# nonl4331/raytracing-rust

Measured on NVIDIA B200. Metric: Mrays/s, higher is better.
Workload: dtype f32

## Files before the change

### raytracing-rust_b200/csrc/context.cu

```cuda
#include <cstdarg>
#include <cstring>
#include <new>

#include "ptb_internal.h"

namespace ptb {

static thread_local std::string g_create_error;

int32_t set_error(Ctx* c, int32_t code, const char* fmt, ...) {
  char buf[512];
  va_list ap;
  va_start(ap, fmt);
  vsnprintf(buf, sizeof buf, fmt, ap);
  va_end(ap);
  if (c) c->last_error = buf;
  else g_create_error = buf;
  return code;
}
int32_t check_cuda(Ctx* c, cudaError_t e, const char* what) {
  if (e == cudaSuccess) return PTB_OK;
  const int32_t code = e == cudaErrorMemoryAllocation ? PTB_ERR_OOM : PTB_ERR_CUDA;
  return set_error(c, code, "CUDA error %d (%s) in %s", (int)e, cudaGetErrorString(e), what);
}
// ... 32 lines not shown
  if (!out) return PTB_ERR_INVALID;
  *out = nullptr;
  int n = 0;
  cudaError_t e = cudaGetDeviceCount(&n);
  if (e != cudaSuccess || n == 0)
    return set_error(nullptr, PTB_ERR_CUDA, "no CUDA device available (%s); ptb200 has no CPU fallback",
                     e == cudaSuccess ? "device count is 0" : cudaGetErrorString(e));
  if (device < 0 || device >= n) return set_error(nullptr, PTB_ERR_INVALID, "device %d out of range [0,%d)", device, n);
  ptb_ctx* ctx = new (std::nothrow) ptb_ctx();
  if (!ctx) return PTB_ERR_OOM;
  Ctx* c = &ctx->c;
  c->device = device;
  auto fail = [&](cudaError_t err, const char* what) {
    int32_t rc = set_error(nullptr, PTB_ERR_CUDA, "%s: %s", what, cudaGetErrorString(err));
    delete ctx;
    return rc;
  };
  if ((e = cudaSetDevice(device)) != cudaSuccess) return fail(e, "cudaSetDevice");
  cudaDeviceProp prop;
  if ((e = cudaGetDeviceProperties(&prop, device)) != cudaSuccess) return fail(e, "cudaGetDeviceProperties");
  if (prop.major < 10) {
    int32_t rc = set_error(nullptr, PTB_ERR_CUDA, "device %d is sm_%d%d; ptb200 is built for sm_100a only", device, prop.major,
                           prop.minor);
    delete ctx;
    return rc;
  }
  c->sm_count = prop.multiProcessorCount;
  c->dev.trace_burst = 8;
  c->dev.trace_fetch_threshold = 8;
  c->dev.trace_prim_bias = 0;
  if (const char* e = getenv("PTB_TRACE_PRIM_BIAS")) { int v = atoi(e); if (v >= 0 && v <= 32) c->dev.trace_prim_bias = v; }
  if (const char* e = getenv("PTB_TRACE_BURST")) { int v = atoi(e); if (v >= 1 && v <= 64) c->dev.trace_burst = v; }
  if (const char* e = getenv("PTB_TRACE_FETCH")) { int v = atoi(e); if (v >= 1 && v <= 32) c->dev.trace_fetch_threshold = v; }
  if ((e = cudaStreamCreateWithFlags(&c->stream, cudaStreamNonBlocking)) != cudaSuccess) return fail(e, "cudaStreamCreate");
  c->own_stream = true;
  if ((e = cudaEventCreate(&c->ev_a)) != cudaSuccess) return fail(e, "cudaEventCreate");
  if ((e = cudaEventCreate(&c->ev_b)) != cudaSuccess) return fail(e, "cudaEventCreate");
  if ((e = cudaEventCreate(&c->ev_iter)) != cudaSuccess) return fail(e, "cudaEventCreate");
  *out = ctx;
  return PTB_OK;
}

int32_t ptb_destroy(ptb_ctx* ctx) {
  if (!ctx) return PTB_OK;
  Ctx* c = &ctx->c;
  cudaSetDevice(c->device);
  if (c->stream) cudaStreamSynchronize(c->stream);
  if (c->h_counters) cudaFreeHost(c->h_counters);
  if (c->h_sah) cudaFreeHost(c->h_sah);
  for (float* h : c->h_pass)
    if (h) cudaFreeHost(h);
  if (c->ev_a) cudaEventDestroy(c->ev_a);
  if (c->ev_b) cudaEventDestroy(c->ev_b);
  if (c->ev_iter) cudaEventDestroy(c->ev_iter);
  for (int b = 0; b < 2; ++b) {
    if (c->ev_in[b]) cudaEventDestroy(c->ev_in[b]);
    if (c->ev_kernel[b]) cudaEventDestroy(c->ev_kernel[b]);
    if (c->ev_out[b]) cudaEventDestroy(c->ev_out[b]);
  }
  for (cudaEvent_t e : c->ev_head_done) if (e) cudaEventDestroy(e);
  for (cudaEvent_t e : c->ev_tail_done) if (e) cudaEventDestroy(e);
  for (cudaEvent_t e : c->ev_ring) if (e) cudaEventDestroy(e);
  if (c->s_tail) { cudaStreamSynchronize(c->s_tail); cudaStreamDestroy(c->s_tail); }
  if (c->s_work2) { cudaStreamSynchronize(c->s_work2); cudaStreamDestroy(c->s_work2); }
  if (c->ev_fork) cudaEventDestroy(c->ev_fork);
  if (c->ev_join) cudaEventDestroy(c->ev_join);
// ... 514 lines not shown
```

### raytracing-rust_b200/csrc/lbvh_build.cu

```cuda
#include <cstdarg>
#include <cstring>

#include "ptb_internal.h"

namespace ptb {

__device__ __forceinline__ uint32_t float_flip(float f) {
  uint32_t u = __float_as_uint(f);
  return (u & 0x80000000u) ? ~u : (u | 0x80000000u);
}
__device__ __forceinline__ float float_unflip(uint32_t u) {
  return __uint_as_float((u & 0x80000000u) ? (u & 0x7FFFFFFFu) : ~u);
}
__device__ __forceinline__ uint32_t expand_bits10(uint32_t v) {
  v = (v * 0x00010001u) & 0xFF0000FFu;
  v = (v * 0x00000101u) & 0x0F00F00Fu;
  v = (v * 0x00000011u) & 0xC30C30C3u;
  v = (v * 0x00000005u) & 0x49249249u;
  return v;
}
__device__ __forceinline__ uint32_t quantise10(float c, float cmin, float ext) {
  float n = ext > 0.0f ? (c - cmin) / ext : 0.0f;
  float s = fminf(fmaxf(n * 1024.0f, 0.0f), 1023.0f);
  return (uint32_t)s;
// ... 752 lines not shown
  if (rc != PTB_OK) return rc;
  PTB_CUDA_TRY(c, cudaEventRecord(c->ev_b, st));
  PTB_CUDA_TRY(c, cudaStreamSynchronize(st));
  PTB_CUDA_TRY(c, cudaGetLastError());
  float ms = 0.f;
  cudaEventElapsedTime(&ms, c->ev_a, c->ev_b);
  c->stats.build_ms = ms;
  if (PTB_QNODES)
    for (int k = 0; k < 3; ++k) { c->dev.q_min[k] = h_qframe[k]; c->dev.q_step[k] = h_qframe[3 + k]; }
  c->dev.lights = c->d_lights.as<uint32_t>();
  c->dev.n_lights = nl;
  c->committed = true;
  return PTB_OK;
}

int32_t build_scene(Ctx* c, uint32_t build_flags) {
  if (build_flags & PTB_BUILD_REFIT) return refit_scene(c, build_flags);
  c->refittable = false;
  {
    int32_t rc = commit_tables(c);
    if (rc != PTB_OK) return rc;
  }
  const size_t ns = c->n_spheres, nt = c->n_tris;
  const size_t n = ns + nt;
  cudaStream_t st = c->stream;

  c->n_prims = n;
  c->n_nodes = n == 0 ? 0 : (n == 1 ? 1 : n - 1);
  c->dev.n_prims = (uint32_t)n;
  c->dev.n_lights = 0;
  c->dev.geom = nullptr; c->dev.normals = nullptr; c->dev.slot_prim = nullptr; c->dev.slot_mat = nullptr;
  c->dev.nodes = nullptr; c->dev.qnodes = nullptr; c->dev.lights = nullptr; c->dev.cw_nodes = nullptr;
  c->wide = false;
  if (n == 0) {
    c->committed = true;
    c->refittable = true;
    c->topo_spheres = ns;
    c->topo_tris = nt;
    c->stats.build_ms = 0.0;
    return PTB_OK;
  }

  DevBuf &raw_spheres = c->d_raw_spheres, &raw_tris = c->d_raw_tris;
  DevBuf &bmin = c->scratch[0], &bmax = c->scratch[1], &bounds = c->scratch[2], &keys_a = c->scratch[3], &keys_b = c->scratch[4],
         &vals_a = c->scratch[5], &vals_b = c->scratch[6], &hist = c->scratch[7], &leaf_parent = c->d_leaf_parent,
         &nbmin = c->scratch[9], &nbmax = c->scratch[10], &flags = c->scratch[11], &prim_slot = c->d_prim_slot,
         &d_light_prims = c->scratch[12], &d_light_tmp = c->scratch[13], &d_light_out = c->scratch[14], &d_qframe = c->scratch[15];
  const uint32_t n32 = (uint32_t)n, ns32 = (uint32_t)ns, nt32 = (uint32_t)nt;
  PTB_CUDA_TRY(c, bmin.reserve(n * 16));
  PTB_CUDA_TRY(c, bmax.reserve(n * 16));
  PTB_CUDA_TRY(c, bounds.reserve(12 * 4));
  PTB_CUDA_TRY(c, keys_a.reserve(n * 4));
  PTB_CUDA_TRY(c, keys_b.reserve(n * 4));
  PTB_CUDA_TRY(c, vals_a.reserve(n * 4));
  PTB_CUDA_TRY(c, vals_b.reserve(n * 4));
  PTB_CUDA_TRY(c, hist.reserve(radix_sort_hist_words(n32) * 4));
  PTB_CUDA_TRY(c, leaf_parent.reserve(n * 4));
  PTB_CUDA_TRY(c, nbmin.reserve(c->n_nodes * 16));
  PTB_CUDA_TRY(c, nbmax.reserve(c->n_nodes * 16));
  PTB_CUDA_TRY(c, flags.reserve(c->n_nodes * 4));
  PTB_CUDA_TRY(c, prim_slot.reserve(n * 4));
  PTB_CUDA_TRY(c, d_light_prims.reserve(n * 4));
  PTB_CUDA_TRY(c, d_light_tmp.reserve(n * 4));
  PTB_CUDA_TRY(c, d_light_out.reserve(8));
  PTB_CUDA_TRY(c, c->d_nodes.reserve(c->n_nodes * sizeof(BvhNode)));
  if (PTB_QNODES) PTB_CUDA_TRY(c, c->d_qnodes.reserve(c->n_nodes * 32));
// ... 81 lines not shown
    const int32_t rcw = build_wide(c, bi, final_prim.as<uint32_t>());
    if (rcw != PTB_OK) return rcw;
    slot_order = final_prim.as<uint32_t>();
    PTB_CUDA_TRY(c, cudaMemcpyAsync(c->d_prim_sorted.p, va, n * 4, cudaMemcpyDeviceToDevice, st));
  }
  k_gather<<<gn, T, 0, st>>>(raw_spheres.as<ptb_sphere>(), ns32, raw_tris.as<ptb_triangle>(), n32, slot_order,
                             c->d_materials.as<DevMaterial>(), (uint32_t)c->materials.size(), c->d_geom.as<float4>(),
                             c->d_normals.as<float4>(),
                             c->d_slot_mat.as<uint32_t>(), prim_slot.as<uint32_t>());
  c->stats.kernel_launches += 1;
  PTB_CUDA_TRY(c, cudaMemcpyAsync(c->d_morton.p, ka, n * 4, cudaMemcpyDeviceToDevice, st));
  PTB_CUDA_TRY(c, cudaMemcpyAsync(c->d_slot_prim.p, slot_order, n * 4, cudaMemcpyDeviceToDevice, st));
  uint32_t nl = 0;
  {
    const int32_t rcl = light_list(c, ns32, &nl);
    if (rcl != PTB_OK) return rcl;
  }
  PTB_CUDA_TRY(c, cudaEventRecord(c->ev_b, st));
  PTB_CUDA_TRY(c, cudaStreamSynchronize(st));
  PTB_CUDA_TRY(c, cudaGetLastError());
  float ms = 0.f;
  cudaEventElapsedTime(&ms, c->ev_a, c->ev_b);
  c->stats.build_ms = ms;

  c->dev.geom = c->d_geom.as<float4>();
  c->dev.normals = c->d_normals.as<float4>();
  c->dev.slot_prim = c->d_slot_prim.as<uint32_t>();
  c->dev.slot_mat = c->d_slot_mat.as<uint32_t>();
  c->dev.nodes = c->d_nodes.as<BvhNode>();
  c->dev.qnodes = (wide || !PTB_QNODES) ? nullptr : c->d_qnodes.as<uint4>();
  for (int k = 0; k < 3; ++k) { c->dev.q_min[k] = h_qframe[k]; c->dev.q_step[k] = h_qframe[3 + k]; }
  c->dev.cw_nodes = wide ? c->d_cw_nodes.as<CwNode>() : nullptr;
  c->wide = wide;
  c->sah = sah;
  if (!wide) c->n_cw_nodes = 0;
  c->dev.lights = c->d_lights.as<uint32_t>();
  c->dev.n_lights = nl;
  c->committed = true;
  c->refittable = true;
  c->topo_spheres = ns;
  c->topo_tris = nt;
  return PTB_OK;
}

}
```

### raytracing-rust_b200/csrc/ptb_common.cuh

```cuda
#pragma once
#include <cuda_runtime.h>
#include <stdint.h>

#include "../../include/ptb200.h"

namespace ptb {

#define PTB_DEV __device__ __forceinline__
#define PTB_HD __host__ __device__ __forceinline__

constexpr float kPi = 3.14159265358979323846f;
constexpr float kTau = 6.28318530717958647692f;
constexpr float kEpsRt = 3.0e-4f;
constexpr float kF32Eps = 1.1920929e-7f;
#ifndef PTB_QNODES
#define PTB_QNODES 0
#endif
constexpr uint32_t kSphereBit = 0x40000000u;
constexpr uint32_t kSlotMask = 0x3FFFFFFFu;
constexpr uint32_t kNone = 0xFFFFFFFFu;

struct v3 {
  float x, y, z;
};
// ... 231 lines not shown
    const float phi = atan2f(direction.y, direction.x) + kPi;
    const float theta = acosf(direction.z);
    const float uvx = phi / (2.0f * kPi), uvy = theta / kPi;
    const uint32_t dim0 = width - 1u, dim1 = height - 1u;
    const uint32_t x_pixel = sat_index((float)dim0 * uvx, dim0), y_pixel = sat_index((float)dim1 * uvy, dim1);
    const uint32_t index = 3u * (y_pixel * (dim0 + 1u) + x_pixel);
    return mk(words.f(index), words.f(index + 1u), words.f(index + 2u));
  }
  if (kind == PTB_TEX_PERLIN) return 0.5f * mk(1.0f, 1.0f, 1.0f) * (1.0f + perlin_noise(words, point));
  return mk(1.0f, 1.0f, 1.0f);
}

struct DevScene {
  const float4* geom;
  const float4* normals;
  const uint32_t* slot_prim;
  const uint32_t* slot_mat;
  const BvhNode* nodes;
  const uint4* qnodes;
  float q_min[3], q_step[3];
  const CwNode* cw_nodes;
  const DevMaterial* materials;
  const DevTexture* textures;
  const float* tex_data;
  const uint32_t* lights;
  uint32_t n_prims, n_lights;
  uint32_t sky_tex, sky_rx, sky_ry;
  const float* sky_ycdf;
  const float* sky_ypdf;
  const float* sky_xcdf;
  const float* sky_xpdf;
  v3 cam_origin, cam_lower_left, cam_horizontal, cam_vertical;
  int trace_burst, trace_fetch_threshold, trace_prim_bias;
};

}
```

### raytracing-rust_b200/csrc/ptb_coop.cuh

```cuda
#pragma once
#include "ptb_intersect.cuh"

namespace ptb {

constexpr uint32_t kCoopRays = 16;
constexpr uint32_t kCoopTagMask = 31u;
#ifndef PTB_COOP_CAP
#define PTB_COOP_CAP 1024
#endif
constexpr uint32_t kCoopCap = PTB_COOP_CAP;
constexpr uint32_t kCoopSoft = kCoopCap - 96u;

#ifdef PTB_TAIL_STATS
__device__ unsigned long long g_tail_stats[16] = {0, 0, 0, 0, 0, 0, 0, 0, 0, ~0ull, 0, 0, 0, 0, 0, 0};
#define PTB_TS(i, v) atomicAdd(&g_tail_stats[i], (unsigned long long)(v))
#else
#define PTB_TS(i, v) do { } while (0)
#endif

struct CoopRay {
  float ox, oy, oz, dx, dy, dz, shx, shy, shz;
  uint32_t swap_xz;
  float ax, ay, az, lx, ly, lz, hx, hy, hz;
  uint32_t exclude;
};
struct CoopWarp {
  unsigned long long best[kCoopRays];
  uint32_t ref[kCoopRays];
  CoopRay ray[kCoopRays];
  uint2 stack[kCoopCap];
};

PTB_DEV void coop_set_ray(const DevScene& sc, CoopWarp& cw, uint32_t j, const Ray& ray, float tmax, uint32_t exclude) {
  const BinRayCtx s = make_bin_ray(sc, ray);
  CoopRay& r = cw.ray[j];
  r.ox = ray.o.x; r.oy = ray.o.y; r.oz = ray.o.z;
  r.dx = ray.d.x; r.dy = ray.d.y; r.dz = ray.d.z;
  r.shx = ray.shear.x; r.shy = ray.shear.y; r.shz = ray.shear.z;
#if PTB_QNODES
  r.ax = s.a.x; r.ay = s.a.y; r.az = s.a.z;
  r.lx = s.b_lo.x; r.ly = s.b_lo.y; r.lz = s.b_lo.z;
  r.hx = s.b_hi.x; r.hy = s.b_hi.y; r.hz = s.b_hi.z;
  r.swap_xz = (ray.swap_xz ? 1u : 0u) | (s.sn_x == kSelHigh ? 2u : 0u) | (s.sn_y == kSelHigh ? 4u : 0u) | (s.sn_z == kSelHigh ? 8u : 0u);
#else
  r.ax = s.dinv.x; r.ay = s.dinv.y; r.az = s.dinv.z;
  r.lx = s.c_lo.x; r.ly = s.c_lo.y; r.lz = s.c_lo.z;
  r.hx = s.c_hi.x; r.hy = s.c_hi.y; r.hz = s.c_hi.z;
  r.swap_xz = ray.swap_xz ? 1u : 0u;
#endif
  r.exclude = exclude;
  cw.best[j] = ((unsigned long long)__float_as_uint(tmax) << 32) | 0xFFFFFFFFull;
  cw.ref[j] = kNone;
}

PTB_DEV uint32_t coop_key(float tkey, uint32_t j) { return (__float_as_uint(fmaxf(tkey, 0.0f)) & ~kCoopTagMask) | j; }

template <bool ANYHIT>
PTB_DEV void coop_trace(const DevScene& sc, CoopWarp& cw, uint32_t n_rays) {
  const uint32_t lane = threadIdx.x & 31u;
  const uint32_t lt = (1u << lane) - 1u;
  uint32_t top = 0;
  if (sc.n_prims) {
    if (lane < n_rays) cw.stack[lane] = make_uint2(0u, lane);
    top = n_rays;
  }
  __syncwarp();
#ifdef PTB_TAIL_STATS
  if (lane == 0u) PTB_TS(5, 1);
  unsigned long long ts_t0;
  asm volatile("mov.u64 %0, %%globaltimer;" : "=l"(ts_t0));
#endif
  while (top) {
    const uint32_t n = top > kCoopSoft ? 1u : (top < 32u ? top : 32u);
    const uint32_t base = top - n;
    bool has = lane < n;
    uint2 e = make_uint2(0u, 0u);
    if (has) e = cw.stack[base + lane];
    top = base;
    __syncwarp();
    const uint32_t j = e.y & kCoopTagMask;
    float bt = 0.0f;
    if (has) {
      bt = __uint_as_float((uint32_t)(cw.best[j] >> 32));
      has = __uint_as_float(e.y & ~kCoopTagMask) <= bt;
    }
#ifdef PTB_TAIL_STATS
    {
      const uint32_t mh = __ballot_sync(0xffffffffu, has);
      if (lane == 0u) { PTB_TS(6, 1); PTB_TS(7, __popc(mh)); PTB_TS(12, n - __popc(mh)); }
    }
#endif
    const bool leaf = has && (e.x & PTB_LEAF_BIT);
    const bool node = has && !leaf;
    float4 a = make_float4(0.f, 0.f, 0.f, 0.f), b = a, c = a;
    uint4 qa = make_uint4(0u, 0u, 0u, 0u), qb = qa;
    uint32_t orig = 0u;
    if (node) {
#if PTB_QNODES
      ldg256u(sc.qnodes + 2u * (size_t)e.x, qa, qb);
#else
      float4 d;
      ldg256(sc.nodes + e.x, a, b);
      ldg256(reinterpret_cast<const float4*>(sc.nodes + e.x) + 2, c, d);
      qb.z = __float_as_uint(d.x);
      qb.w = __float_as_uint(d.y);
#endif
// ... 29 lines not shown
      const bool hr = box_entry(b.z, b.w, c.x, c.y, c.z, c.w, s, bt, tr);
#endif
      const uint32_t cl = qb.z, cr = qb.w;
      if (hl && hr) {
        const bool right_first = tr < tl;
        p0 = right_first ? make_uint2(cl, coop_key(tl, j)) : make_uint2(cr, coop_key(tr, j));
        p1 = right_first ? make_uint2(cr, coop_key(tr, j)) : make_uint2(cl, coop_key(tl, j));
        cnt = 2u;
      } else if (hl || hr) {
        p0 = hl ? make_uint2(cl, coop_key(tl, j)) : make_uint2(cr, coop_key(tr, j));
        cnt = 1u;
      }
    } else if (leaf) {
      const uint32_t slot = e.x & kSlotMask;
      if (!ANYHIT || slot != r.exclude) {
        Ray ray;
        ray.o = mk(r.ox, r.oy, r.oz);
        ray.d = mk(r.dx, r.dy, r.dz);
        ray.shear = mk(r.shx, r.shy, r.shz);
        ray.dinv = mk(0.0f, 0.0f, 0.0f);
        ray.swap_xz = (r.swap_xz & 1u) != 0u;
        const float t = (e.x & kSphereBit) ? sphere_t(ray, from4(a), a.w) : triangle_t(ray, from4(a), from4(b), from4(c));
        if (t > 0.0f && (ANYHIT ? t < bt : t <= bt)) {
          packed = ((unsigned long long)__float_as_uint(t) << 32) | (unsigned long long)orig;
          candidate = packed < atomicMin(&cw.best[j], packed);
        }
      }
    }
    const uint32_t m1 = __ballot_sync(0xffffffffu, cnt >= 1u), m2 = __ballot_sync(0xffffffffu, cnt == 2u);
    const uint32_t pos = top + (uint32_t)__popc(m1 & lt) + (uint32_t)__popc(m2 & lt);
    if (cnt >= 1u) cw.stack[pos] = p0;
    if (cnt == 2u) cw.stack[pos + 1u] = p1;
    top += (uint32_t)__popc(m1) + (uint32_t)__popc(m2);
    __syncwarp();
    if (candidate && cw.best[j] == packed) cw.ref[j] = e.x & ~PTB_LEAF_BIT;
  }
  __syncwarp();
#ifdef PTB_TAIL_STATS
  unsigned long long ts_t1;
  asm volatile("mov.u64 %0, %%globaltimer;" : "=l"(ts_t1));
  if (lane == 0u) PTB_TS(13, ts_t1 - ts_t0);
#endif
}

}
```

### raytracing-rust_b200/csrc/ptb_internal.h

```cpp
#pragma once
#include <cuda_runtime.h>

#include <cstdio>
#include <map>
#include <string>
#include <vector>

#include "ptb_common.cuh"

namespace ptb {

struct DevBuf {
  void* p = nullptr;
  size_t bytes = 0;
  DevBuf() {}
  DevBuf(const DevBuf&) = delete;
  DevBuf& operator=(const DevBuf&) = delete;
  ~DevBuf() { release(); }
  void release() {
    if (p) cudaFree(p);
    p = nullptr;
    bytes = 0;
  }
  cudaError_t alloc(size_t n) {
// ... 67 lines not shown
  bool refittable = false;
  size_t topo_spheres = 0, topo_tris = 0;
  DevBuf d_geom, d_normals, d_slot_prim, d_slot_mat, d_nodes, d_qnodes, d_cw_nodes, d_prim_sorted, d_morton, d_materials, d_textures, d_tex_data, d_lights;
  DevBuf d_sky_ycdf, d_sky_ypdf, d_sky_xcdf, d_sky_xpdf;
  uint64_t n_prims = 0, n_nodes = 0, n_cw_nodes = 0;
  bool wide = false;
  uint32_t cw_max_leaf = 3;
  DevBuf cw_scratch[10];
  bool sah = false;
  uint32_t sah_levels = 0;
  DevBuf sah_scratch[12];
  uint32_t* h_sah = nullptr;

  DevBuf d_accum;
  float* accum_target = nullptr;
  DevBuf d_pass;
  float* h_pass[2] = {nullptr, nullptr};
  size_t h_pass_floats = 0;
  uint32_t accum_w = 0, accum_h = 0;
  uint64_t accum_samples = 0;
  DevBuf d_pool_mem, d_prev, d_queues, d_shadow, d_counters, d_windows;
  DevBuf d_pool_mem2, d_prev2, d_queues2, d_shadow2, d_counters2, d_windows2;
  cudaStream_t s_tail = nullptr;
  cudaStream_t s_work2 = nullptr;
  cudaEvent_t ev_fork = nullptr, ev_join = nullptr;
  cudaEvent_t ev_head_done[2] = {}, ev_tail_done[2] = {};
  cudaEvent_t ev_ring[8] = {};
  PathPool pool;
  size_t pool_budget_bytes = 0;
  WaveCounters* h_counters = nullptr;
  cudaEvent_t ev_a = nullptr, ev_b = nullptr, ev_iter = nullptr;
  cudaEvent_t ev_prof[64] = {};
  bool opt_time_kernels = false, opt_count_traversal = false;

  DevBuf d_rays, d_hits, d_rays2, d_hits2;
  DevBuf d_index, d_index2;
  DevBuf d_hit_sort;
  cudaStream_t s_in = nullptr, s_out = nullptr;
  cudaEvent_t ev_in[2] = {}, ev_kernel[2] = {}, ev_out[2] = {};

  ptb_stats stats{};
};

int32_t set_error(Ctx* c, int32_t code, const char* fmt, ...);
int32_t check_cuda(Ctx* c, cudaError_t e, const char* what);

int32_t build_scene(Ctx* c, uint32_t flags);
int32_t tree_sah_cost(Ctx* c, double* cost);
struct CwBuildInputs {
  const BvhNode* nodes;
  const uint2* range;
  const float4 *nbmin, *nbmax;
  const float4 *bmin, *bmax;
  const uint32_t* prim_sorted;
  uint32_t n_prims;
};
int32_t build_wide(Ctx* c, const CwBuildInputs& in, uint32_t* final_prim);
int32_t exclusive_scan(Ctx* c, uint32_t* data, uint32_t n, uint32_t* block_sum, uint32_t* total_out);
void scan_block_sums(Ctx* c, uint32_t* block_sum, uint32_t n_blocks, uint32_t* total_out);
struct SahBuildInputs {
  const float4 *bmin, *bmax;
  const uint32_t* box6;
  uint32_t *order_a, *order_b;
  BvhNode* nodes;
  uint32_t* leaf_parent;
  uint32_t n_prims, n_spheres;
};
int32_t build_sah(Ctx* c, const SahBuildInputs& in, const uint32_t** order_out);
int32_t reserve_sah(Ctx* c, uint32_t n_prims);
void radix_sort_pairs(Ctx* c, uint32_t*& ka, uint32_t*& va, uint32_t*& kb, uint32_t*& vb, uint32_t n, int passes, uint32_t* hist);
size_t radix_sort_hist_words(uint32_t n);
int32_t render_wavefront(Ctx* c, const ptb_render_opts& o, ptb_progress_fn progress, void* user);
int32_t launch_closest_hit(Ctx* c, const void* d_rays, size_t n, void* d_hits);
int32_t launch_visibility(Ctx* c, const void* d_rays, const void* d_index, size_t n, void* d_out);
void free_render_state(Ctx* c);
int32_t sampler_hook(Ctx* c, const ptb_sampler_query& q, size_t n, const float* dirs_in, float* dirs_out, float* pdf_out);

}

// ... 10 lines not shown
```

### raytracing-rust_b200/csrc/ptb_traverse.cuh

```cuda
#pragma once
#include "ptb_coop.cuh"
#include "ptb_cwbvh.cuh"
#include "ptb_intersect.cuh"

namespace ptb {

#ifndef PTB_PREFETCH
#define PTB_PREFETCH 0
#endif
PTB_DEV void prefetch_l1(const void* p) { asm volatile("prefetch.global.L1 [%0];" ::"l"(p)); }
constexpr int kStackDepth = 64;
#ifndef PTB_LEAF_QUEUE
#define PTB_LEAF_QUEUE 1
#endif
constexpr uint32_t kLeafQueue = PTB_LEAF_QUEUE;

struct TraceResult {
  float t;
  uint32_t ref;
};

PTB_DEV void load_node(const BvhNode* __restrict__ nodes, uint32_t idx, float4& n0, float4& n1, float4& n2, uint4& n3) {
  float4 t;
  ldg256(nodes + idx, n0, n1);
// ... 222 lines not shown
  PTB_DEV static bool done(const State& s) { return s.done(); }
  template <bool COUNT>
  PTB_DEV static void node_step(const DevScene& sc, const RayCtx& rc, State& s, Scratch& k, uint32_t& n) {
    cw_node_step<COUNT>(sc.cw_nodes, rc, s, k.stack, n);
  }
  template <bool ANYHIT, bool COUNT>
  PTB_DEV static void prim_step(const DevScene& sc, const Ray& ray, State& s, Scratch& k, uint32_t exclude, uint32_t& n) {
    cw_prim_step<ANYHIT, COUNT>(sc, ray, s, k.stack, exclude, n);
  }
  PTB_DEV static TraceResult result(const State& s) {
    TraceResult r;
    r.t = 0.0f;
    r.ref = kNone;
    if (s.best_ref != kNone) { r.t = s.best_t; r.ref = s.best_ref; }
    return r;
  }
};

#ifdef PTB_DRAIN_STATS
__device__ unsigned long long g_drain[6] = {~0ull, 0ull, ~0ull, 0ull, 0ull, 0ull};
PTB_DEV unsigned long long drain_now() {
  unsigned long long t;
  asm volatile("mov.u64 %0, %%globaltimer;" : "=l"(t));
  return t;
}
#endif
#ifdef PTB_LANE_STATS
__device__ unsigned long long g_lane_stats[8];
#define PTB_LS(i, v) do { if (lane == 0u) ls[i] += (v); } while (0)
#else
#define PTB_LS(i, v) do { } while (0)
#endif

template <class TR, bool ANYHIT, bool COUNT, class Fetch, class Retire>
PTB_DEV void persistent_trace(const DevScene& sc, uint32_t n, uint32_t* head, Fetch& fetch, Retire& retire,
                              uint32_t& cnt_nodes, uint32_t& cnt_prims, uint32_t& cnt_rays) {
  const uint32_t lane = threadIdx.x & 31u;
  typename TR::Scratch scratch;
  typename TR::State st;
  typename TR::RayCtx rc = TR::idle();
  TR::init(st, rc, 0u, 0.0f);
  Ray ray;
  ray.o = ray.d = ray.dinv = ray.shear = mk(0.0f, 0.0f, 0.0f);
  ray.swap_xz = false;
  uint32_t exclude = kNone;
  bool has_ray = false, exhausted = false;
  const uint32_t total_warps = gridDim.x * (blockDim.x >> 5);
  uint32_t cap = (n + total_warps - 1u) / total_warps;
  cap = cap < 1u ? 1u : (cap > 32u ? 32u : cap);
  const uint32_t fetch_below = (uint32_t)sc.trace_fetch_threshold < cap ? (uint32_t)sc.trace_fetch_threshold : cap;
#ifdef PTB_LANE_STATS
  unsigned long long ls[8] = {0, 0, 0, 0, 0, 0, 0, 0};
#endif
#ifdef PTB_DRAIN_STATS
  if (threadIdx.x == 0u) atomicMin(&g_drain[2], drain_now());
#endif
  for (;;) {
    bool node_ready = has_ray && TR::node_ready(st);
    const bool leaf_ready = has_ray && TR::leaf_ready(st);
    const uint32_t m_node = __ballot_sync(0xffffffffu, node_ready);
    const uint32_t m_leaf = __ballot_sync(0xffffffffu, leaf_ready);
    PTB_LS(0, 1);
    PTB_LS(1, __popc(m_node | m_leaf));
    if ((uint32_t)__popc(m_node | m_leaf) < (exhausted ? 1u : fetch_below)) {
      PTB_LS(6, 1);
      const bool fin = has_ray && !node_ready && !leaf_ready;
      retire(fin, TR::result(st), ray);
      if (fin) has_ray = false;
      if (exhausted) {
        if (!__any_sync(0xffffffffu, has_ray)) break;
        continue;
      }
      uint32_t idle = __ballot_sync(0xffffffffu, !has_ray);
      if (cap < 32u) {
        const uint32_t busy = 32u - (uint32_t)__popc(idle);
        const uint32_t allow = busy < cap ? cap - busy : 0u;
        const uint32_t cut = __fns(idle, 0u, (int)allow + 1);
        if (cut != 0xffffffffu) idle &= (1u << cut) - 1u;
      }
      if (idle) {
        const uint32_t leader = __ffs(idle) - 1u, want = __popc(idle);
        uint32_t base = 0;
        if (lane == leader) base = atomicAdd(head, want);
        base = __shfl_sync(0xffffffffu, base, leader);
        const uint32_t mine = base + __popc(idle & ((1u << lane) - 1u));
        if (((idle >> lane) & 1u) && mine < n) {
          float tmax = __int_as_float(0x7f800000);
          fetch(mine, ray, tmax, exclude);
          rc = TR::make(sc, ray);
          TR::init(st, rc, sc.n_prims, tmax);
          has_ray = true;
          if (COUNT) ++cnt_rays;
        }
        if (base + want >= n) exhausted = true;
#ifdef PTB_DRAIN_STATS
        if (lane == leader && base + want >= n) atomicMin(&g_drain[0], drain_now());
#endif
      }
      continue;
    }
    const int n_node = __popc(m_node), n_blocked = __popc(m_leaf & ~m_node), n_leaf = __popc(m_leaf);
    const bool do_node = sc.trace_prim_bias ? (n_node >= n_blocked * sc.trace_prim_bias) : (n_node >= n_leaf);
    if (do_node) {
      PTB_LS(2, 1);
      PTB_LS(3, n_node);
#pragma unroll 1
      for (int burst = 0; burst < sc.trace_burst && node_ready; ++burst) {
        TR::template node_step<COUNT>(sc, rc, st, scratch, cnt_nodes);
        node_ready = TR::node_ready(st);
#ifdef PTB_LANE_STATS
        atomicAdd(&g_lane_stats[7], 1ull);
#endif
      }
    } else if (leaf_ready) {
      TR::template prim_step<ANYHIT, COUNT>(sc, ray, st, scratch, exclude, cnt_prims);
    }
#ifdef PTB_LANE_STATS
    if (!do_node) { PTB_LS(4, 1); PTB_LS(5, n_leaf); }
#endif
  }
#ifdef PTB_LANE_STATS
  if (lane == 0u)
    for (int i = 0; i < 7; ++i) atomicAdd(&g_lane_stats[i], ls[i]);
#endif
#ifdef PTB_DRAIN_STATS
  if (lane == 0u) atomicMax(&g_drain[1], drain_now());
#endif
}

template <class TR, bool ANYHIT>
PTB_DEV TraceResult trace_lane(const DevScene& sc, const Ray& ray, float tmax, uint32_t exclude, typename TR::Scratch& scratch) {
  typename TR::State st;
  const typename TR::RayCtx rc = TR::make(sc, ray);
  TR::init(st, rc, sc.n_prims, tmax);
  uint32_t unused = 0;
  while (!TR::done(st)) {
    if (TR::node_ready(st)) TR::template node_step<false>(sc, rc, st, scratch, unused);
    else TR::template prim_step<ANYHIT, false>(sc, ray, st, scratch, exclude, unused);
  }
  return TR::result(st);
}

}
```

### raytracing-rust_b200/csrc/wavefront.cu

```cuda
#include "ptb_internal.h"
#include "ptb_traverse.cuh"
#include "ptb_packet.cuh"

namespace ptb {

struct RenderParams {
  uint32_t width, height, npix;
  uint32_t row_begin;
  uint32_t tile_w, tile_h;
  uint32_t group;
  uint32_t dir_bins;
  uint32_t sample_offset;
  uint32_t method, max_depth, rr_threshold;
  uint32_t k0, k1;
};

struct Queues {
  uint32_t* active[2];
  uint32_t* free_slots;
  uint32_t* kind[kNumKinds];
  float4* shadow;
  uint32_t* win_count;
  uint32_t* win_prefix;
  uint32_t* seg_total;
// ... 1090 lines not shown
        if (bins[k] != kBinDead) q.active[0][hist[bins[k]] + offs[k]] = first_slot + tid * kWinItems + k;
      buf ^= 1u;
    }
  }
}

struct ShadowFetch {
  const Queues& q;
  float4 contrib;
  PTB_DEV void operator()(uint32_t i, Ray& ray, float& tmax, uint32_t& exclude) {
    const float4* e = q.shadow + 3u * (size_t)i;
    const float4 o = e[0], d = e[1];
    contrib = e[2];
    ray = make_ray(from4(o), from4(d));
    tmax = o.w;
    exclude = __float_as_uint(d.w);
  }
};
struct ShadowRetire {
  const PathPool& pool;
  const ShadowFetch& f;
  PTB_DEV void operator()(bool fin, const TraceResult& tr, const Ray&) {
    if (fin && tr.ref == kNone) {
      const uint32_t slot = __float_as_uint(f.contrib.w);
      float4 ra = pool.col[4u * (size_t)slot + 1u];
      ra.x += f.contrib.x; ra.y += f.contrib.y; ra.z += f.contrib.z;
      pool.col[4u * (size_t)slot + 1u] = ra;
    }
  }
};
#ifndef PTB_SHADOW_MIN_BLOCKS
#define PTB_SHADOW_MIN_BLOCKS 1
#endif
template <class TR>
__global__ void __launch_bounds__(256, PTB_SHADOW_MIN_BLOCKS) k_shadow(DevScene sc, PathPool pool, Queues q, WaveCounters* wc) {
  uint32_t a = 0, b = 0, r = 0;
  ShadowFetch fetch{q, make_float4(0.f, 0.f, 0.f, 0.f)};
  ShadowRetire retire{pool, fetch};
  persistent_trace<TR, true, false>(sc, (uint32_t)wc->shadow_pair, &wc->shadow_head, fetch, retire, a, b, r);
}

PTB_DEV unsigned long long global_timer_ns() {
  unsigned long long t;
  asm volatile("mov.u64 %0, %%globaltimer;" : "=l"(t));
  return t;
}
template <int METHOD, bool FULL>
PTB_DEV void tail_shade(const DevScene& sc, const PathPool& pool, const RenderParams& rp, uint32_t slot, const Ray& ray,
                        const TraceResult& tr, ShadeOut& so) {
  stg256(pool.ray + 4u * (size_t)slot, make_float4(ray.o.x, ray.o.y, ray.o.z, tr.t),
         make_float4(ray.d.x, ray.d.y, ray.d.z, __uint_as_float(tr.ref)));
  so.fin_L = mk(0.0f, 0.0f, 0.0f);
  shade_path<METHOD, FULL>(sc, pool, rp, slot, false, kNoCamera, so);
}
PTB_DEV void tail_add_nee(const PathPool& pool, uint32_t slot, const ShadeOut& so) {
  float4 ra = pool.col[4u * (size_t)slot + 1u];
  ra.x += so.sh_c.x; ra.y += so.sh_c.y; ra.z += so.sh_c.z;
  pool.col[4u * (size_t)slot + 1u] = ra;
}
PTB_DEV void tail_finish(float* __restrict__ accum, const Queues& q, uint32_t slot, const ShadeOut& so) {
  if (so.contributes) {
    atomicAdd(accum + 3u * (size_t)so.fin_pixel + 0, so.fin_L.x);
    atomicAdd(accum + 3u * (size_t)so.fin_pixel + 1, so.fin_L.y);
    atomicAdd(accum + 3u * (size_t)so.fin_pixel + 2, so.fin_L.z);
  }
  q.bin[slot] = (uint8_t)kBinDead;
}

constexpr uint32_t kCoopMinPrims = 4096u;
#ifndef PTB_TAIL_WARPS
#define PTB_TAIL_WARPS 4
#endif
constexpr int kTailThreads = 32 * PTB_TAIL_WARPS;
template <class TR, int METHOD, bool FULL>
__global__ void __launch_bounds__(kTailThreads)
k_tail(DevScene sc, PathPool pool, Queues q, WaveCounters* wc, RenderParams rp, float* __restrict__ accum, uint32_t depth) {
  if (wc->tail_iter != depth) return;
  const uint32_t n = wc->n_tail;
  if (threadIdx.x == 0u) atomicMin(&wc->tail_t0, global_timer_ns());
#ifdef PTB_TAIL_STATS
  if (threadIdx.x == 0u) atomicMin(&g_tail_stats[9], global_timer_ns());
#endif
  constexpr bool COOP = TR::kCoop;
  __shared__ CoopWarp s_coop[COOP ? PTB_TAIL_WARPS : 1];
  const uint32_t lane = threadIdx.x & 31u, warp = threadIdx.x >> 5;
  unsigned long long c_bounce = 0, c_sky = 0, c_light = 0, c_ref = 0, c_paths = 0;
  const uint32_t mask = n <= 1u ? 0u : (1u << (32 - __clz(n - 1u))) - 1u;
  if (COOP && sc.n_prims >= kCoopMinPrims) {
    CoopWarp& cw = s_coop[warp];
    const uint32_t lt = (1u << lane) - 1u;
    uint32_t slot = kNone;
    bool exhausted = false;
    for (;;) {
      if (slot == kNone && !exhausted) {
        const uint32_t t = atomicAdd(&wc->tail_head, 1u);
        if (t < n) {
          uint32_t i = t;
          do { i = (i * 0x9E3779B1u) & mask; } while (i >= n);
          slot = q.active[0][i];
        } else {
          exhausted = true;
        }
// ... 339 lines not shown
  return c->wide ? trace_kernel_of<CwTrav>(count, dense, camera) : trace_kernel_of<BinTrav>(count, dense, camera);
}
static const void* shadow_kernel(const Ctx* c) { return c->wide ? (const void*)k_shadow<CwTrav> : (const void*)k_shadow<BinTrav>; }
static const void* api_kernel(const Ctx* c, bool count) {
  if (c->wide) return count ? (const void*)k_closest_hit_api<CwTrav, true> : (const void*)k_closest_hit_api<CwTrav, false>;
  return count ? (const void*)k_closest_hit_api<BinTrav, true> : (const void*)k_closest_hit_api<BinTrav, false>;
}
static const void* visibility_kernel(const Ctx* c, bool chi) {
  if (c->wide) return chi ? (const void*)k_visibility_api<CwTrav, true> : (const void*)k_visibility_api<CwTrav, false>;
  return chi ? (const void*)k_visibility_api<BinTrav, true> : (const void*)k_visibility_api<BinTrav, false>;
}
template <class TR>
static const void* tail_kernel_of(bool mis, bool full) {
  if (mis) return full ? (const void*)k_tail<TR, PTB_METHOD_MIS, true> : (const void*)k_tail<TR, PTB_METHOD_MIS, false>;
  return full ? (const void*)k_tail<TR, PTB_METHOD_NAIVE, true> : (const void*)k_tail<TR, PTB_METHOD_NAIVE, false>;
}
static cudaError_t launch_trace(const void* fn, int grid, cudaStream_t st, const DevScene& sc, const PathPool& pool, const Queues& q,
                                WaveCounters* wc, const RenderParams& rp, unsigned long long first) {
  void* args[] = {(void*)&sc, (void*)&pool, (void*)&q, (void*)&wc, (void*)&rp, (void*)&first};
  return cudaLaunchKernel(fn, dim3((unsigned)grid), dim3(256), args, 0, st);
}
static cudaError_t launch_shadow(const void* fn, int grid, cudaStream_t st, const DevScene& sc, const PathPool& pool, const Queues& q,
                                 WaveCounters* wc) {
  void* args[] = {(void*)&sc, (void*)&pool, (void*)&q, (void*)&wc};
  return cudaLaunchKernel(fn, dim3((unsigned)grid), dim3(256), args, 0, st);
}

static int persistent_grid(Ctx* c, const void* kernel, int threads) {
  int per_sm = 0;
  if (cudaOccupancyMaxActiveBlocksPerMultiprocessor(&per_sm, kernel, threads, 0) != cudaSuccess || per_sm < 1) per_sm = 1;
  return c->sm_count * per_sm;
}

static int32_t prepare_batch(Ctx* c, const float4* r4, size_t n, uint32_t** head, unsigned long long** counts,
                             const uint32_t** order) {
  if (n > 0xFFFFFFF0ull) return set_error(c, PTB_ERR_INVALID, "too many rays in one batch");
  PTB_CUDA_TRY(c, c->d_counters.reserve(sizeof(WaveCounters) + 64));
  char* scratch = c->d_counters.as<char>() + sizeof(WaveCounters);
  *head = reinterpret_cast<uint32_t*>(scratch);
  *counts = reinterpret_cast<unsigned long long*>(scratch + 8);
  PTB_CUDA_TRY(c, cudaMemsetAsync(scratch, 0, 24, c->stream));
  *order = nullptr;
  bool sort = n >= (1u << 16) && c->n_prims > 0;
  if (const char* e = getenv("PTB_HIT_SORT")) sort = sort && atoi(e) != 0;
  if (sort) {
    const uint32_t n32 = (uint32_t)n;
    PTB_CUDA_TRY(c, c->d_hit_sort.reserve(((size_t)n32 * 4 + radix_sort_hist_words(n32)) * 4));
    uint32_t* w = c->d_hit_sort.as<uint32_t>();
    uint32_t *ka = w, *va = w + n, *kb = w + 2 * n, *vb = w + 3 * n, *hist = w + 4 * n;
    k_ray_sort_keys<<<(n32 + 255u) / 256u, 256, 0, c->stream>>>(c->dev, r4, n32, ka, va);
    c->stats.kernel_launches += 1;
    radix_sort_pairs(c, ka, va, kb, vb, n32, 3, hist);
    *order = va;
  }
  return PTB_OK;
}

int32_t launch_closest_hit(Ctx* c, const void* d_rays, size_t n, void* d_hits) {
  if (n == 0) return PTB_OK;
  const float4* r4 = reinterpret_cast<const float4*>(d_rays);
  uint4* h4 = reinterpret_cast<uint4*>(d_hits);
  uint32_t* head;
  unsigned long long* counts;
  const uint32_t* order;
  const int32_t rc = prepare_batch(c, r4, n, &head, &counts, &order);
  if (rc != PTB_OK) return rc;
// ... 667 lines not shown
```

Measured before the change: 4926.

## Drain straggler rays with warp-cooperative traversal using a global frontier pool

Once the ray queue is exhausted, a warp whose live ray count falls below a threshold claims a per-SM global-memory frontier slot and switches the remaining rays to cooperative warp traversal. This is meant to cut the long tail where few active lanes keep a warp busy. The change also raises the minimum blocks per SM for the binned shadow kernel. In exchange it adds global-memory frontier traffic, atomic slot claiming, a new context allocation, and possible register pressure.

```diff
diff --git a/raytracing-rust_b200/csrc/context.cu b/raytracing-rust_b200/csrc/context.cu
--- a/raytracing-rust_b200/csrc/context.cu
+++ b/raytracing-rust_b200/csrc/context.cu
@@ -88,6 +88,13 @@
   if (const char* e = getenv("PTB_TRACE_PRIM_BIAS")) { int v = atoi(e); if (v >= 0 && v <= 32) c->dev.trace_prim_bias = v; }
   if (const char* e = getenv("PTB_TRACE_BURST")) { int v = atoi(e); if (v >= 1 && v <= 64) c->dev.trace_burst = v; }
   if (const char* e = getenv("PTB_TRACE_FETCH")) { int v = atoi(e); if (v >= 1 && v <= 32) c->dev.trace_fetch_threshold = v; }
+  c->drain_lanes = 8;
+  if (const char* e = getenv("PTB_DRAIN_COOP")) { int v = atoi(e); if (v >= 0 && v <= 32) c->drain_lanes = (uint32_t)v; }
+  if (const char* e = getenv("PTB_DRAIN_MIN_PRIMS")) { long v = atol(e); if (v >= 0) c->drain_min_prims = v; }
+  if (c->drain_lanes) {
+    int32_t rc = ptb::alloc_drain_pool(c);
+    if (rc != PTB_OK) { delete ctx; return rc; }
+  }
   if ((e = cudaStreamCreateWithFlags(&c->stream, cudaStreamNonBlocking)) != cudaSuccess) return fail(e, "cudaStreamCreate");
   c->own_stream = true;
   if ((e = cudaEventCreate(&c->ev_a)) != cudaSuccess) return fail(e, "cudaEventCreate");
diff --git a/raytracing-rust_b200/csrc/lbvh_build.cu b/raytracing-rust_b200/csrc/lbvh_build.cu
--- a/raytracing-rust_b200/csrc/lbvh_build.cu
+++ b/raytracing-rust_b200/csrc/lbvh_build.cu
@@ -808,6 +808,7 @@
   c->dev.geom = nullptr; c->dev.normals = nullptr; c->dev.slot_prim = nullptr; c->dev.slot_mat = nullptr;
   c->dev.nodes = nullptr; c->dev.qnodes = nullptr; c->dev.lights = nullptr; c->dev.cw_nodes = nullptr;
   c->wide = false;
+  set_drain(c);
   if (n == 0) {
     c->committed = true;
     c->refittable = true;
@@ -955,6 +956,7 @@
   for (int k = 0; k < 3; ++k) { c->dev.q_min[k] = h_qframe[k]; c->dev.q_step[k] = h_qframe[3 + k]; }
   c->dev.cw_nodes = wide ? c->d_cw_nodes.as<CwNode>() : nullptr;
   c->wide = wide;
+  set_drain(c);
   c->sah = sah;
   if (!wide) c->n_cw_nodes = 0;
   c->dev.lights = c->d_lights.as<uint32_t>();
diff --git a/raytracing-rust_b200/csrc/ptb_common.cuh b/raytracing-rust_b200/csrc/ptb_common.cuh
--- a/raytracing-rust_b200/csrc/ptb_common.cuh
+++ b/raytracing-rust_b200/csrc/ptb_common.cuh
@@ -287,6 +287,9 @@
   const float* sky_xpdf;
   v3 cam_origin, cam_lower_left, cam_horizontal, cam_vertical;
   int trace_burst, trace_fetch_threshold, trace_prim_bias;
-};
-
-}
+  uint32_t drain_lanes, drain_pool_sms;
+  void* drain_pool;
+  uint32_t* drain_claim;
+};
+
+}
diff --git a/raytracing-rust_b200/csrc/ptb_coop.cuh b/raytracing-rust_b200/csrc/ptb_coop.cuh
--- a/raytracing-rust_b200/csrc/ptb_coop.cuh
+++ b/raytracing-rust_b200/csrc/ptb_coop.cuh
@@ -1,5 +1,8 @@
 #pragma once
 #include "ptb_intersect.cuh"
+#ifdef PTB_DEBUG
+#include <cassert>
+#endif
 
 namespace ptb {
 
@@ -9,7 +12,7 @@
 #define PTB_COOP_CAP 1024
 #endif
 constexpr uint32_t kCoopCap = PTB_COOP_CAP;
-constexpr uint32_t kCoopSoft = kCoopCap - 96u;
+constexpr uint32_t kCoopMinPrims = 4096u;
 
 #ifdef PTB_TAIL_STATS
 __device__ unsigned long long g_tail_stats[16] = {0, 0, 0, 0, 0, 0, 0, 0, 0, ~0ull, 0, 0, 0, 0, 0, 0};
@@ -24,14 +27,19 @@
   float ax, ay, az, lx, ly, lz, hx, hy, hz;
   uint32_t exclude;
 };
-struct CoopWarp {
+template <uint32_t CAP>
+struct CoopFrontier {
+  static_assert(CAP >= 128u, "the overflow rule needs 96 entries of headroom above a soft limit of at least 32");
+  static constexpr uint32_t kCap = CAP, kSoft = CAP - 96u;
   unsigned long long best[kCoopRays];
   uint32_t ref[kCoopRays];
   CoopRay ray[kCoopRays];
-  uint2 stack[kCoopCap];
+  uint2 stack[CAP];
 };
+typedef CoopFrontier<kCoopCap> CoopWarp;
 
-PTB_DEV void coop_set_ray(const DevScene& sc, CoopWarp& cw, uint32_t j, const Ray& ray, float tmax, uint32_t exclude) {
+template <uint32_t CAP>
+PTB_DEV void coop_set_ray(const DevScene& sc, CoopFrontier<CAP>& cw, uint32_t j, const Ray& ray, float tmax, uint32_t exclude) {
   const BinRayCtx s = make_bin_ray(sc, ray);
   CoopRay& r = cw.ray[j];
   r.ox = ray.o.x; r.oy = ray.o.y; r.oz = ray.o.z;
@@ -55,8 +63,8 @@
 
 PTB_DEV uint32_t coop_key(float tkey, uint32_t j) { return (__float_as_uint(fmaxf(tkey, 0.0f)) & ~kCoopTagMask) | j; }
 
-template <bool ANYHIT>
-PTB_DEV void coop_trace(const DevScene& sc, CoopWarp& cw, uint32_t n_rays) {
+template <bool ANYHIT, uint32_t CAP>
+PTB_DEV void coop_trace(const DevScene& sc, CoopFrontier<CAP>& cw, uint32_t n_rays) {
   const uint32_t lane = threadIdx.x & 31u;
   const uint32_t lt = (1u << lane) - 1u;
   uint32_t top = 0;
@@ -71,7 +79,7 @@
   asm volatile("mov.u64 %0, %%globaltimer;" : "=l"(ts_t0));
 #endif
   while (top) {
-    const uint32_t n = top > kCoopSoft ? 1u : (top < 32u ? top : 32u);
+    const uint32_t n = top > CoopFrontier<CAP>::kSoft ? 1u : (top < 32u ? top : 32u);
     const uint32_t base = top - n;
     bool has = lane < n;
     uint2 e = make_uint2(0u, 0u);
@@ -167,6 +175,9 @@
     if (cnt >= 1u) cw.stack[pos] = p0;
     if (cnt == 2u) cw.stack[pos + 1u] = p1;
     top += (uint32_t)__popc(m1) + (uint32_t)__popc(m2);
+#ifdef PTB_DEBUG
+    assert(top <= CAP);
+#endif
     __syncwarp();
     if (candidate && cw.best[j] == packed) cw.ref[j] = e.x & ~PTB_LEAF_BIT;
   }
diff --git a/raytracing-rust_b200/csrc/ptb_internal.h b/raytracing-rust_b200/csrc/ptb_internal.h
--- a/raytracing-rust_b200/csrc/ptb_internal.h
+++ b/raytracing-rust_b200/csrc/ptb_internal.h
@@ -123,6 +123,9 @@
   cudaEvent_t ev_a = nullptr, ev_b = nullptr, ev_iter = nullptr;
   cudaEvent_t ev_prof[64] = {};
   bool opt_time_kernels = false, opt_count_traversal = false;
+  uint32_t drain_lanes = 0;
+  int64_t drain_min_prims = -1;
+  DevBuf d_drain_pool;
 
   DevBuf d_rays, d_hits, d_rays2, d_hits2;
   DevBuf d_index, d_index2;
@@ -136,6 +139,8 @@
 int32_t set_error(Ctx* c, int32_t code, const char* fmt, ...);
 int32_t check_cuda(Ctx* c, cudaError_t e, const char* what);
 
+void set_drain(Ctx* c);
+int32_t alloc_drain_pool(Ctx* c);
 int32_t build_scene(Ctx* c, uint32_t flags);
 int32_t tree_sah_cost(Ctx* c, double* cost);
 struct CwBuildInputs {
diff --git a/raytracing-rust_b200/csrc/ptb_traverse.cuh b/raytracing-rust_b200/csrc/ptb_traverse.cuh
--- a/raytracing-rust_b200/csrc/ptb_traverse.cuh
+++ b/raytracing-rust_b200/csrc/ptb_traverse.cuh
@@ -278,10 +278,72 @@
 #define PTB_LS(i, v) do { } while (0)
 #endif
 
+#ifndef PTB_DRAIN_CAP
+#define PTB_DRAIN_CAP 256
+#endif
+typedef CoopFrontier<PTB_DRAIN_CAP> DrainFrontier;
+constexpr uint32_t kDrainPerSm = 64;
+PTB_DEV uint32_t sm_id() {
+  uint32_t r;
+  asm volatile("mov.u32 %0, %%smid;" : "=r"(r));
+  return r;
+}
+PTB_DEV uint32_t hw_warp_id() {
+  uint32_t r;
+  asm volatile("mov.u32 %0, %%warpid;" : "=r"(r));
+  return r;
+}
+
+PTB_DEV uint32_t drain_claim(const DevScene& sc) {
+  const uint32_t base = (sm_id() % sc.drain_pool_sms) * kDrainPerSm, first = hw_warp_id();
+  for (uint32_t k = 0; k < kDrainPerSm; ++k) {
+    const uint32_t i = base + ((first + k) & (kDrainPerSm - 1u));
+    if (atomicCAS(sc.drain_claim + i, 0u, 1u) == 0u) return i;
+  }
+  return ~0u;
+}
+
+template <bool ANYHIT>
+PTB_DEV TraceResult drain_coop(const DevScene& sc, uint32_t got, uint32_t live, const Ray& ray, float best_t,
+                               uint32_t best_ref, uint32_t exclude) {
+  const uint32_t lane = threadIdx.x & 31u, lt = (1u << lane) - 1u;
+  DrainFrontier& f = static_cast<DrainFrontier*>(sc.drain_pool)[got];
+  TraceResult tr;
+  tr.t = 0.0f;
+  tr.ref = kNone;
+  for (uint32_t todo = live; todo;) {
+    const bool mine = ((todo >> lane) & 1u) && (uint32_t)__popc(todo & lt) < kCoopRays;
+    const uint32_t bm = __ballot_sync(0xffffffffu, mine);
+    const uint32_t r = (uint32_t)__popc(bm & lt);
+    if (mine) {
+      coop_set_ray(sc, f, r, ray, best_t, ANYHIT ? exclude : kNone);
+      if (!ANYHIT && best_ref != kNone) {
+        f.best[r] = ((unsigned long long)__float_as_uint(best_t) << 32) | __ldg(sc.slot_prim + (best_ref & kSlotMask));
+        f.ref[r] = best_ref & ~PTB_LEAF_BIT;
+      }
+    }
+    __syncwarp();
+    coop_trace<ANYHIT>(sc, f, (uint32_t)__popc(bm));
+    if (mine) {
+      tr.ref = f.ref[r];
+      tr.t = tr.ref == kNone ? 0.0f : __uint_as_float((uint32_t)(f.best[r] >> 32));
+    }
+    __syncwarp();
+    todo &= ~bm;
+  }
+  if (lane == 0u) {
+    __threadfence();
+    atomicExch(sc.drain_claim + got, 0u);
+  }
+  return tr;
+}
+
 template <class TR, bool ANYHIT, bool COUNT, class Fetch, class Retire>
 PTB_DEV void persistent_trace(const DevScene& sc, uint32_t n, uint32_t* head, Fetch& fetch, Retire& retire,
                               uint32_t& cnt_nodes, uint32_t& cnt_prims, uint32_t& cnt_rays) {
   const uint32_t lane = threadIdx.x & 31u;
+  const uint32_t drain = TR::kCoop && !COUNT ? sc.drain_lanes : 0u;
+  uint32_t drain_live = 0u, drain_frontier = ~0u;
   typename TR::Scratch scratch;
   typename TR::State st;
   typename TR::RayCtx rc = TR::idle();
@@ -308,42 +370,53 @@
     const uint32_t m_leaf = __ballot_sync(0xffffffffu, leaf_ready);
     PTB_LS(0, 1);
     PTB_LS(1, __popc(m_node | m_leaf));
-    if ((uint32_t)__popc(m_node | m_leaf) < (exhausted ? 1u : fetch_below)) {
+    if ((uint32_t)__popc(m_node | m_leaf) < (exhausted ? drain + 1u : fetch_below)) {
       PTB_LS(6, 1);
       const bool fin = has_ray && !node_ready && !leaf_ready;
       retire(fin, TR::result(st), ray);
       if (fin) has_ray = false;
       if (exhausted) {
-        if (!__any_sync(0xffffffffu, has_ray)) break;
+        const uint32_t live = __ballot_sync(0xffffffffu, has_ray);
+        if (!live) break;
+        if (drain) {
+          uint32_t got = ~0u;
+          if (lane == 0u) got = drain_claim(sc);
+          got = __shfl_sync(0xffffffffu, got, 0);
+          if (got != ~0u) {
+            drain_live = live;
+            drain_frontier = got;
+            break;
+          }
+        }
+      } else {
+        uint32_t idle = __ballot_sync(0xffffffffu, !has_ray);
+        if (cap < 32u) {
+          const uint32_t busy = 32u - (uint32_t)__popc(idle);
+          const uint32_t allow = busy < cap ? cap - busy : 0u;
+          const uint32_t cut = __fns(idle, 0u, (int)allow + 1);
+          if (cut != 0xffffffffu) idle &= (1u << cut) - 1u;
+        }
+        if (idle) {
+          const uint32_t leader = __ffs(idle) - 1u, want = __popc(idle);
+          uint32_t base = 0;
+          if (lane == leader) base = atomicAdd(head, want);
+          base = __shfl_sync(0xffffffffu, base, leader);
+          const uint32_t mine = base + __popc(idle & ((1u << lane) - 1u));
+          if (((idle >> lane) & 1u) && mine < n) {
+            float tmax = __int_as_float(0x7f800000);
+            fetch(mine, ray, tmax, exclude);
+            rc = TR::make(sc, ray);
+            TR::init(st, rc, sc.n_prims, tmax);
+            has_ray = true;
+            if (COUNT) ++cnt_rays;
+          }
+          if (base + want >= n) exhausted = true;
+#ifdef PTB_DRAIN_STATS
+          if (lane == leader && base + want >= n) atomicMin(&g_drain[0], drain_now());
+#endif
+        }
         continue;
       }
-      uint32_t idle = __ballot_sync(0xffffffffu, !has_ray);
-      if (cap < 32u) {
-        const uint32_t busy = 32u - (uint32_t)__popc(idle);
-        const uint32_t allow = busy < cap ? cap - busy : 0u;
-        const uint32_t cut = __fns(idle, 0u, (int)allow + 1);
-        if (cut != 0xffffffffu) idle &= (1u << cut) - 1u;
-      }
-      if (idle) {
-        const uint32_t leader = __ffs(idle) - 1u, want = __popc(idle);
-        uint32_t base = 0;
-        if (lane == leader) base = atomicAdd(head, want);
-        base = __shfl_sync(0xffffffffu, base, leader);
-        const uint32_t mine = base + __popc(idle & ((1u << lane) - 1u));
-        if (((idle >> lane) & 1u) && mine < n) {
-          float tmax = __int_as_float(0x7f800000);
-          fetch(mine, ray, tmax, exclude);
-          rc = TR::make(sc, ray);
-          TR::init(st, rc, sc.n_prims, tmax);
-          has_ray = true;
-          if (COUNT) ++cnt_rays;
-        }
-        if (base + want >= n) exhausted = true;
-#ifdef PTB_DRAIN_STATS
-        if (lane == leader && base + want >= n) atomicMin(&g_drain[0], drain_now());
-#endif
-      }
-      continue;
     }
     const int n_node = __popc(m_node), n_blocked = __popc(m_leaf & ~m_node), n_leaf = __popc(m_leaf);
     const bool do_node = sc.trace_prim_bias ? (n_node >= n_blocked * sc.trace_prim_bias) : (n_node >= n_leaf);
@@ -365,6 +438,12 @@
     if (!do_node) { PTB_LS(4, 1); PTB_LS(5, n_leaf); }
 #endif
   }
+  if constexpr (TR::kCoop && !COUNT) {
+    if (drain_frontier != ~0u) {
+      const TraceResult tr = drain_coop<ANYHIT>(sc, drain_frontier, drain_live, ray, st.best_t, st.best_ref, exclude);
+      retire(((drain_live >> lane) & 1u) != 0u, tr, ray);
+    }
+  }
 #ifdef PTB_LANE_STATS
   if (lane == 0u)
     for (int i = 0; i < 7; ++i) atomicAdd(&g_lane_stats[i], ls[i]);
diff --git a/raytracing-rust_b200/csrc/wavefront.cu b/raytracing-rust_b200/csrc/wavefront.cu
--- a/raytracing-rust_b200/csrc/wavefront.cu
+++ b/raytracing-rust_b200/csrc/wavefront.cu
@@ -1146,8 +1146,11 @@
 #ifndef PTB_SHADOW_MIN_BLOCKS
 #define PTB_SHADOW_MIN_BLOCKS 1
 #endif
+#ifndef PTB_SHADOW_BIN_MIN_BLOCKS
+#define PTB_SHADOW_BIN_MIN_BLOCKS 3
+#endif
 template <class TR>
-__global__ void __launch_bounds__(256, PTB_SHADOW_MIN_BLOCKS) k_shadow(DevScene sc, PathPool pool, Queues q, WaveCounters* wc) {
+__global__ void __launch_bounds__(256, TR::kCoop ? PTB_SHADOW_BIN_MIN_BLOCKS : PTB_SHADOW_MIN_BLOCKS) k_shadow(DevScene sc, PathPool pool, Queues q, WaveCounters* wc) {
   uint32_t a = 0, b = 0, r = 0;
   ShadowFetch fetch{q, make_float4(0.f, 0.f, 0.f, 0.f)};
   ShadowRetire retire{pool, fetch};
@@ -1181,7 +1184,6 @@
   q.bin[slot] = (uint8_t)kBinDead;
 }
 
-constexpr uint32_t kCoopMinPrims = 4096u;
 #ifndef PTB_TAIL_WARPS
 #define PTB_TAIL_WARPS 4
 #endif
@@ -1587,6 +1589,20 @@
   return c->sm_count * per_sm;
 }
 
+void set_drain(Ctx* c) {
+  const uint64_t min_prims = c->drain_min_prims < 0 ? kCoopMinPrims : (uint64_t)c->drain_min_prims;
+  c->dev.drain_lanes = (!c->wide && c->n_prims >= min_prims) ? c->drain_lanes : 0u;
+}
+int32_t alloc_drain_pool(Ctx* c) {
+  const size_t n = (size_t)c->sm_count * kDrainPerSm, claims = n * sizeof(DrainFrontier);
+  PTB_CUDA_TRY(c, c->d_drain_pool.alloc(claims + n * sizeof(uint32_t)));
+  PTB_CUDA_TRY(c, cudaMemset(c->d_drain_pool.as<char>() + claims, 0, n * sizeof(uint32_t)));
+  c->dev.drain_pool = c->d_drain_pool.p;
+  c->dev.drain_claim = reinterpret_cast<uint32_t*>(c->d_drain_pool.as<char>() + claims);
+  c->dev.drain_pool_sms = (uint32_t)c->sm_count;
+  return PTB_OK;
+}
+
 static int32_t prepare_batch(Ctx* c, const float4* r4, size_t n, uint32_t** head, unsigned long long** counts,
                              const uint32_t** order) {
   if (n > 0xFFFFFFF0ull) return set_error(c, PTB_ERR_INVALID, "too many rays in one batch");
```

New measurement: 4901, median of 6. About the same (-0.5%).
